# huster-wgm/SRCGAN

Hardware: AMD Instinct MI355X
Metric: paired SR-CycleGAN train images/sec at x4 256->1024 (higher is better)
Workload: dtype bf16; 1 GPU; Sat2Aerx4 paired G+D step (BASELINE configs[1]): 23-block RRDB generator + 3-layer PatchGAN, 3x256x256->3x1024x1024, batch 16/GPU; per_gpu_batch=16, global_batch=16, parallelism=dp1, gradient_exchange=none (1 rank)

## Files before the change

srcgan_amd/csrc/wgrad_dense.hip:

```cpp
#include "common.h"
#include <type_traits>
#include <stdlib.h>

struct WdSeg { int g0, g1; float* grad; float* bias; int Cin; float alpha; };
struct WdP {
    const void* dy; const void* x; float* slab;
    int B, H, W, G, C, dycoff, xcoff;
    long dypix, dyplane, xpix, xplane;
    int g_base;
    int cin_lim[4];
    int nsplit, tiles_x, tiles_y, ntiles, ncit, want_bias;
    unsigned long long* trace;
};
struct WdRedP {
    const float* slab; int nsplit, ncit, COT, g_base, nseg; WdSeg seg[8]; int accumulate;
};

typedef __attribute__((address_space(3))) s16x4 lds_s16x4_;
__device__ __forceinline__ bf16x8 tr_frag2(const char* p0, const char* p1) {
    s16x4 lo = __builtin_amdgcn_ds_read_tr16_b64_v4i16((lds_s16x4_*)(p0));
    s16x4 hi = __builtin_amdgcn_ds_read_tr16_b64_v4i16((lds_s16x4_*)(p1));
    typedef __attribute__((ext_vector_type(8))) short s16x8;
    s16x8 v = {lo[0], lo[1], lo[2], lo[3], hi[0], hi[1], hi[2], hi[3]};
    return __builtin_bit_cast(bf16x8, v);
}

static __device__ __attribute__((aligned(64))) unsigned int wd_zero_page[16];
template <typename T>
__device__ __forceinline__ size_t wd_chan_off(int c, long plane) {
    constexpr int KCE = DT<T>::KCE;
    return (size_t)(c / KCE) * plane + (size_t)(c % KCE) * sizeof(T);
}
typedef const __attribute__((address_space(1))) void* wd_gptr_t;
typedef __attribute__((address_space(3))) void* wd_lptr_t;

template <typename T, int MT, int NT, int TH>
__global__ __launch_bounds__(MT * NT * 64) void wgrad_dense_k(const WdP p) {
    using D = DT<T>;
    constexpr int NW = MT * NT, TW = 32, NTAP = 9;
    constexpr int IHT = TH + 2, IWT = TW + 2;
    constexpr int PB = 32 * (int)sizeof(T), PPP = PB / 16, PXP = 64 / PPP;
    constexpr int DPX = TH * TW, XPX = IHT * IWT;
    constexpr int DPP = (DPX + PXP - 1) / PXP, XPP = (XPX + PXP - 1) / PXP;
    constexpr int DBYTES = DPP * 1024, XBYTES = XPP * 1024;
    constexpr int NPIECE = MT * DPP + NT * XPP, SBYTES = MT * DBYTES + NT * XBYTES;
    constexpr int IPW = (NPIECE + NW - 1) / NW;
    extern __shared__ __attribute__((aligned(1024))) char smem[];

    const int tid = threadIdx.x, lane = tid & 63, wave = tid >> 6, r = lane & 31, h = lane >> 5;
    const int wm = wave / NT, wn = wave % NT;
    const int cit = blockIdx.x, split = blockIdx.y;
    const bool do_bias = wn == 0 && cit == 0 && p.want_bias;
    const char* zp = (const char*)wd_zero_page;

    f32x16 acc[NTAP + 1];
#pragma unroll
    for (int a = 0; a <= NTAP; ++a)
#pragma unroll
        for (int i = 0; i < 16; ++i) acc[a][i] = 0.f;

    const int t_begin = (int)((long)p.ntiles * split / p.nsplit);
    const int t_end = (int)((long)p.ntiles * (split + 1) / p.nsplit);

    auto issue = [&](int t, int stage) {
        int q = t;
        const int tx = q % p.tiles_x; q /= p.tiles_x;
        const int ty = q % p.tiles_y;
        const int b = q / p.tiles_y;
        const int oy0 = ty * TH, ox0 = tx * TW;
        const char* dyb = (const char*)p.dy + (size_t)b * p.H * p.W * p.dypix;
        const char* xb = (const char*)p.x + (size_t)b * p.H * p.W * p.xpix;
        char* ls = smem + stage * SBYTES;
#pragma unroll
        for (int it = 0; it < IPW; ++it) {
            const int pi = it * NW + wave;
            if (IPW * NW != NPIECE && pi >= NPIECE) continue;
            const char* src = zp;
            const int part = lane % PPP, lpx = lane / PPP;
            if (pi < MT * DPP) {
                const int m = pi / DPP, pix = (pi - m * DPP) * PXP + lpx;
                const int oy = oy0 + pix / TW, ox = ox0 + pix % TW;
                const int ch = p.g_base + m * 32 + part * D::EPP;
                if (pix < DPX && oy < p.H && ox < p.W && ch < p.G)
                    src = dyb + (size_t)(oy * p.W + ox) * p.dypix + wd_chan_off<T>(p.dycoff + ch, p.dyplane);
            } else {
                const int pj = pi - MT * DPP, n = pj / XPP, pix = (pj - n * XPP) * PXP + lpx;
                const int iy = pix / IWT, ix = pix - iy * IWT;
                const int gy = oy0 - 1 + iy, gx = ox0 - 1 + ix;
                const int ch = (cit * NT + n) * 32 + part * D::EPP;
                if (pix < XPX && (unsigned)gy < (unsigned)p.H && (unsigned)gx < (unsigned)p.W && ch < p.C)
                    src = xb + (size_t)(gy * p.W + gx) * p.xpix + wd_chan_off<T>(p.xcoff + ch, p.xplane);
            }
            __builtin_amdgcn_global_load_lds((wd_gptr_t)src, (wd_lptr_t)(ls + pi * 1024), 16, 0, 0);
        }
    };

    if (t_begin < t_end) issue(t_begin, 0);
    int stage = 0;
    for (int t = t_begin; t < t_end; ++t, stage ^= 1) {
        __syncthreads();
        if (t + 1 < t_end) issue(t + 1, stage ^ 1);
        const char* my_d = smem + stage * SBYTES + wm * DBYTES;
        const char* my_x = smem + stage * SBYTES + MT * DBYTES + wn * XBYTES;
        if constexpr (std::is_same<T, float>::value) {
#pragma unroll 2
            for (int kk = 0; kk < TH * TW / 2; ++kk) {
                const int pix = 2 * kk + h;
                const int py = pix / TW, px = pix % TW;
                const float a = *(const float*)(my_d + pix * PB + r * 4);
#pragma unroll
                for (int tap = 0; tap < NTAP; ++tap) {
                    const int ky = tap / 3, kx = tap % 3;
                    const float bv = *(const float*)(my_x + ((py + ky) * IWT + px + kx) * PB + r * 4);
                    acc[tap] = __builtin_amdgcn_mfma_f32_32x32x2f32(a, bv, acc[tap], 0, 0, 0);
                }
                if (do_bias) acc[NTAP] = __builtin_amdgcn_mfma_f32_32x32x2f32(a, 1.0f, acc[NTAP], 0, 0, 0);
            }
        } else {
            const int gq = lane >> 4, idx = lane & 15, qq = idx >> 2, pp = idx & 3;
            const int choff = ((gq & 1) * 16 + 4 * pp) * 2;
            const bf16x8 ones = sg_ones16<T>();
#pragma unroll 2
            for (int kk = 0; kk < TH * 2; ++kk) {
                const int py = kk >> 1, xh = (kk & 1) * 16;
                const int px0 = xh + 8 * h + qq;
                const char* ab = my_d + (py * TW + px0) * PB + choff;
                const bf16x8 a = tr_frag2(ab, ab + 4 * PB);
#pragma unroll
                for (int tap = 0; tap < NTAP; ++tap) {
                    const int ky = tap / 3, kx = tap % 3;
                    const char* bb = my_x + ((py + ky) * IWT + px0 + kx) * PB + choff;
                    acc[tap] = sg_mfma16<T>(a, tr_frag2(bb, bb + 4 * PB), acc[tap]);
                }
                if (do_bias) acc[NTAP] = sg_mfma16<T>(a, ones, acc[NTAP]);
            }
        }
    }

    constexpr int COT = 32 * MT, CIT = 32 * NT;
    float* sp = p.slab + ((size_t)split * p.ncit + cit) * (NTAP + 1) * COT * CIT;
#pragma unroll
    for (int tap = 0; tap <= NTAP; ++tap) {
        if (tap == NTAP && !do_bias) continue;
#pragma unroll
        for (int i = 0; i < 16; ++i) {
            const int row = wm * 32 + 8 * (i >> 2) + 4 * h + (i & 3);
            sp[((size_t)tap * COT + row) * CIT + wn * 32 + r] = acc[tap][i];
        }
    }
}

typedef int wd_v4i __attribute__((ext_vector_type(4)));
__device__ __forceinline__ void wd_dma16(const void* base, int voff, int soff, wd_lptr_t lds) {
    const unsigned long long a = (unsigned long long)base;
    wd_v4i rs;
    rs[0] = __builtin_amdgcn_readfirstlane((int)(a & 0xffffffffu));
    rs[1] = __builtin_amdgcn_readfirstlane((int)((a >> 32) & 0xffffu));
    rs[2] = 0x7fffffff;
    rs[3] = 0x00020000;
    const unsigned dst = __builtin_amdgcn_readfirstlane((unsigned)(unsigned long long)lds);
    unsigned keep;
    asm volatile("s_mov_b32 %0, m0\n\ts_mov_b32 m0, %3\n\ts_nop 0\n\tbuffer_load_dwordx4 %1, %2, %4 offen lds\n\ts_mov_b32 m0, %0"
                 : "=&s"(keep) : "v"(voff), "s"(rs), "s"(dst), "s"(soff) : "memory");
}

#ifndef SG_WD_EXP
#define SG_WD_EXP 0
#endif
template <typename T, int MT, int NT, int TH>
__global__ __launch_bounds__(MT * NT * 64) void wgrad_dense_fast_k(const WdP p) {
    using D = DT<T>;
    constexpr int NW = MT * NT, TW = 32, NTAP = 9;
    constexpr int IHT = TH + 2, IWT = TW + 2;
    constexpr int PB = 64, PXP = 16;
    constexpr int DPX = TH * TW, XPX = IHT * IWT;
    constexpr int DPP = (DPX + PXP - 1) / PXP, XPP = (XPX + PXP - 1) / PXP;
    constexpr int DBYTES = DPP * 1024, XBYTES = XPP * 1024;
    constexpr int NPIECE = MT * DPP + NT * XPP, SBYTES = MT * DBYTES + NT * XBYTES;
    constexpr int IPW = (NPIECE + NW - 1) / NW;
    constexpr int OOB = 0x7fffffff;
#ifndef SG_WD_PPK
#define SG_WD_PPK 0
#endif
    constexpr int PPK = SG_WD_PPK ? SG_WD_PPK : 4;
    static_assert(IPW <= 16, "piece classes are packed 4 bits each into two registers");
    extern __shared__ __attribute__((aligned(1024))) char smem[];

    const int tid = threadIdx.x, lane = tid & 63, r = lane & 31, h = lane >> 5;
    const int wave = __builtin_amdgcn_readfirstlane(tid >> 6);
    const int wm = wave / NT, wn = wave % NT;
    int cit, split;
    {
        const int L = blockIdx.x + gridDim.x * blockIdx.y, nwg = gridDim.x * gridDim.y;
        const int xcd = L & 7, j = L >> 3;
        const int full = (nwg >> 3) * 8;
        const int per = nwg >> 3;
        const int pos = L < full ? xcd * per + j : L;
        cit = pos % p.ncit; split = pos / p.ncit;
        if (split >= p.nsplit) return;
    }
    const bool do_bias = wn == 0 && cit == 0 && p.want_bias;
#ifdef SG_WD_NO_SKIP
    const bool useful = true;
#else
    const bool useful = (cit * NT + wn) * 32 < p.cin_lim[wm] || do_bias;
#endif

#ifndef SG_WD_S16
#define SG_WD_S16 1
#endif
    constexpr bool S16 = SG_WD_S16 != 0;
    int voff[IPW]; long soff[IPW];
    unsigned cls[2] = {0u, 0u};
    {
        const int part = lane & 3, lpx = lane >> 2;
#pragma unroll
        for (int it = 0; it < IPW; ++it) {
            const int pi = it * NW + wave;
            int v = OOB; long so = 0;
            if (pi < MT * DPP) {
                const int m = pi / DPP, pix = (pi - m * DPP) * PXP + lpx;
                const int psw = S16 ? part ^ ((((pix % TW) >> 3) & 1) << 1) : part;
                const int ch = p.g_base + m * 32 + psw * D::EPP;
                if (pix < DPX && ch < p.G) v = ((pix / TW) * p.W + pix % TW) * (int)p.dypix + psw * 16;
                so = (long)wd_chan_off<T>(p.dycoff + p.g_base + m * 32, p.dyplane);
            } else if (pi < NPIECE) {
                const int pj = pi - MT * DPP, n = pj / XPP, pix = (pj - n * XPP) * PXP + lpx;
                const int iy = pix / IWT, ix = pix - iy * IWT;
                const int psw = S16 ? part ^ (((ix >> 3) & 1) << 1) : part;
                const int ch = (cit * NT + n) * 32 + psw * D::EPP;
                if (pix < XPX && ch < p.C) v = (iy * p.W + ix) * (int)p.xpix + psw * 16;
                so = (long)wd_chan_off<T>(p.xcoff + (cit * NT + n) * 32, p.xplane);
                cls[it / 8] |= (unsigned)((iy == 0) | ((iy == IHT - 1) << 1) | ((ix == 0) << 2) | ((ix == IWT - 1) << 3)) << (4 * (it % 8));
            }
            voff[it] = v;
            soff[it] = ((long)__builtin_amdgcn_readfirstlane((int)(so >> 32)) << 32) | (unsigned)__builtin_amdgcn_readfirstlane((int)(so & 0xffffffff));
        }
    }

    f32x16 acc[S16 ? 1 : NTAP + 1];
    f32x4 acq[S16 ? NTAP + 1 : 1][2][2];
#pragma unroll
    for (int a = 0; a < (S16 ? 1 : NTAP + 1); ++a)
#pragma unroll
        for (int i = 0; i < 16; ++i) acc[a][i] = 0.f;
#pragma unroll
    for (int a = 0; a < (S16 ? NTAP + 1 : 1); ++a)
#pragma unroll
        for (int i = 0; i < 16; ++i) acq[a][(i >> 3) & 1][(i >> 2) & 1][i & 3] = 0.f;

    const int t_begin = (int)((long)p.ntiles * split / p.nsplit);
    const int t_end = (int)((long)p.ntiles * (split + 1) / p.nsplit);
    int ty = t_begin % p.tiles_y, tx = (t_begin / p.tiles_y) % p.tiles_x, tb = t_begin / (p.tiles_x * p.tiles_y);
    tx = __builtin_amdgcn_readfirstlane(tx); ty = __builtin_amdgcn_readfirstlane(ty); tb = __builtin_amdgcn_readfirstlane(tb);
    const char* dyo = nullptr; const char* xo = nullptr; unsigned clm[2] = {0u, 0u};
    auto origin = [&]() {
        const long px = ((long)tb * p.H + ty * TH) * p.W + tx * TW;
        dyo = (const char*)p.dy + px * p.dypix;
        xo = (const char*)p.x + (px - p.W - 1) * p.xpix;
        const unsigned m = (unsigned)((ty == 0) | ((ty == p.tiles_y - 1) << 1) | ((tx == 0) << 2) | ((tx == p.tiles_x - 1) << 3));
        clm[0] = cls[0] & (m * 0x11111111u); clm[1] = cls[1] & (m * 0x11111111u);
    };
    auto advance = [&]() { if (++ty == p.tiles_y) { ty = 0; if (++tx == p.tiles_x) { tx = 0; ++tb; } } };
    auto piece = [&](int it, int stage) __attribute__((always_inline)) {
        const int pi = it * NW + wave;
        if (IPW * NW != NPIECE && pi >= NPIECE) return;
        int v = ((clm[it / 8] >> (4 * (it % 8))) & 15u) ? OOB : voff[it];
        if (SG_WD_EXP & 8) v = OOB;
        wd_dma16((pi < MT * DPP ? dyo : xo) + soff[it], v, 0, (wd_lptr_t)(smem + stage * SBYTES + pi * 1024));
    };

    if (t_begin < t_end) {
        origin();
#pragma unroll
        for (int it = 0; it < IPW; ++it) piece(it, 0);
    }
    const int gq = lane >> 4, idx = lane & 15, qq = idx >> 2, pp = idx & 3;
    const int choff = ((gq & 1) * 16 + 4 * pp) * 2;
    const bf16x8 ones = sg_ones16<T>();
    int stage = 0;
    for (int t = t_begin; t < t_end; ++t, stage ^= 1) {
#ifdef SG_TRACE
        const unsigned long long t_arr = __builtin_amdgcn_s_memrealtime();
        __builtin_amdgcn_s_waitcnt(0x0f70);
        const unsigned long long t_land = __builtin_amdgcn_s_memrealtime();
#endif
        __builtin_amdgcn_s_waitcnt(0x0f70);
        __syncthreads();
#ifdef SG_TRACE
        if (p.trace && blockIdx.x == 1 && blockIdx.y == 3 && lane == 0 && t - t_begin >= 8 && t - t_begin < 12)
            p.trace[160 + (t - t_begin - 8) * 8 + wave] = t_arr;
        if (p.trace && blockIdx.x == 1 && blockIdx.y == 3 && wave == 0 && lane == 0 && t - t_begin < 40) {
            p.trace[(t - t_begin) * 4 + 0] = t_arr; p.trace[(t - t_begin) * 4 + 1] = t_land; p.trace[(t - t_begin) * 4 + 2] = __builtin_amdgcn_s_memrealtime();
            p.trace[(t - t_begin) * 4 + 3] = __builtin_readcyclecounter();
        }
#endif
        const bool more = t + 1 < t_end;
        if (more) { advance(); origin(); }
        if (!useful) {
            if (more && !(SG_WD_EXP & 1)) {
#pragma unroll
                for (int it = 0; it < IPW; ++it) piece(it, stage ^ 1);
            }
            continue;
        }
        const char* my_d = smem + stage * SBYTES + wm * DBYTES;
        const char* my_x = smem + stage * SBYTES + MT * DBYTES + wn * XBYTES;
#ifndef SG_WD_PD
#define SG_WD_PD 4
#endif
        if constexpr (S16) {
            constexpr int NG = IHT * 3, PDG = 1;
            bf16x8 fa[TH][2], fb[PDG + 1][2];
            const int kq = lane >> 4;
            const int lb = (8 * kq + qq) * PB + (kq & 1) * 32 + 8 * pp;
            const int mk1 = qq + 1 >= 4 ? 32 : 0, mk2 = qq + 2 >= 4 ? 32 : 0;
            auto rd_b = [&](int G) {
                const int i2 = G / 3, kx = G % 3;
                const char* bb = my_x + (i2 * IWT + kx) * PB;
                const int l0 = lb, l1 = lb ^ (kx == 0 ? 0 : kx == 1 ? mk1 : mk2);
                fb[G % (PDG + 1)][0] = tr_frag2(bb + l0, bb + 4 * PB + l1);
                fb[G % (PDG + 1)][1] = tr_frag2(bb + (l0 ^ 32), bb + 4 * PB + (l1 ^ 32));
            };
            auto rd_a = [&](int py) {
                const char* ab = my_d + py * TW * PB;
                fa[py][0] = tr_frag2(ab + lb, ab + 4 * PB + lb);
                fa[py][1] = tr_frag2(ab + (lb ^ 32), ab + 4 * PB + (lb ^ 32));
            };
            rd_a(0); rd_b(0);
#pragma unroll
            for (int G = 0; G < NG; ++G) {
                const int i2 = G / 3, kx = G % 3;
                if (kx == 1 && i2 + 1 < TH) rd_a(i2 + 1);
                if (G + PDG < NG) rd_b(G + PDG);
                if (more) {
#pragma unroll
                    for (int j = 0; j < 2 * PPK; ++j)
                        if (2 * PPK * G + j < IPW) piece(2 * PPK * G + j, stage ^ 1);
                }
                __builtin_amdgcn_sched_barrier(0);
#pragma unroll
                for (int py = 0; py < TH; ++py) {
                    const int ky = i2 - py;
                    if (ky < 0 || ky > 2) continue;
#pragma unroll
                    for (int mb = 0; mb < 2; ++mb)
#pragma unroll
                        for (int nb = 0; nb < 2; ++nb)
                            acq[ky * 3 + kx][mb][nb] = sg_mfma16s<T>(fa[py][mb], fb[G % (PDG + 1)][nb], acq[ky * 3 + kx][mb][nb]);
                }
                if (do_bias && kx == 0 && (i2 == 0 || i2 >= IHT - 2))
#pragma unroll
                    for (int py = (i2 == 0 ? 0 : i2 == IHT - 2 ? 1 : TH / 2); py < (i2 == 0 ? 1 : i2 == IHT - 2 ? TH / 2 : TH); ++py)
#pragma unroll
                        for (int mb = 0; mb < 2; ++mb) acq[NTAP][mb][0] = sg_mfma16s<T>(fa[py][mb], ones, acq[NTAP][mb][0]);
                __builtin_amdgcn_sched_barrier(0);
            }
        } else {
        constexpr int NGRP = IHT * 3 * 2, PD = SG_WD_PD;
        bf16x8 fa[TH][2], fb[PD + 1];
        auto read_b = [&](int G) {
            const int i2 = G / 6, kx = (G % 6) / 2, xh = G % 2;
            const char* bb = my_x + (i2 * IWT + xh * 16 + 8 * h + qq + kx) * PB + choff;
            fb[G % (PD + 1)] = tr_frag2(bb, bb + 4 * PB);
        };
        auto read_a = [&](int py, int xh) {
            const char* ab = my_d + (py * TW + xh * 16 + 8 * h + qq) * PB + choff;
            fa[py][xh] = tr_frag2(ab, ab + 4 * PB);
        };
        read_a(0, 0); read_b(0); read_a(0, 1);
#pragma unroll
        for (int G = 1; G < PD; ++G) read_b(G);
        constexpr int FA_LEAD = 4;
#ifndef SG_WD_PRIO_K
#define SG_WD_PRIO_K 0
#endif
#pragma unroll
        for (int G = 0; G < NGRP; ++G) {
            if (SG_WD_PRIO_K > 0 && wave >= NW / 2) {
                if (G == 0) __builtin_amdgcn_s_setprio(1);
                if (G == SG_WD_PRIO_K) __builtin_amdgcn_s_setprio(0);
            }
            if ((G + FA_LEAD) % 6 < 2 && (G + FA_LEAD) / 6 >= 1 && (G + FA_LEAD) / 6 < TH) read_a((G + FA_LEAD) / 6, (G + FA_LEAD) % 6);
            if (G + PD < NGRP && !(SG_WD_EXP & 4)) read_b(G + PD);
            if (more && !(SG_WD_EXP & 1)) {
#pragma unroll
                for (int j = 0; j < PPK; ++j)
                    if (PPK * G + j < IPW) piece(PPK * G + j, stage ^ 1);
            }
            __builtin_amdgcn_sched_barrier(0);
#ifdef SG_TRACE
            if (G % 5 == 0 && p.trace && blockIdx.x == 1 && blockIdx.y == 3 && lane == 0 && t - t_begin == 10)
                p.trace[192 + wave * 8 + G / 5] = __builtin_amdgcn_s_memrealtime();
#endif
            const int i2 = G / 6, kx = (G % 6) / 2, xh = G % 2;
#pragma unroll
            for (int py = 0; py < TH; ++py) {
                const int ky = i2 - py;
                if (ky < 0 || ky > 2) continue;
                if (!(SG_WD_EXP & 2)) acc[ky * 3 + kx] = sg_mfma16<T>(fa[py][xh], fb[G % (PD + 1)], acc[ky * 3 + kx]);
                else asm volatile("" :: "v"(fa[py][xh]), "v"(fb[G % (PD + 1)]));
            }
            if (do_bias && kx == 0 && (i2 == 0 || i2 >= IHT - 2))
#pragma unroll
                for (int py = (i2 == 0 ? 0 : i2 == IHT - 2 ? 1 : TH / 2); py < (i2 == 0 ? 1 : i2 == IHT - 2 ? TH / 2 : TH); ++py)
                    acc[NTAP] = sg_mfma16<T>(fa[py][xh], ones, acc[NTAP]);
            __builtin_amdgcn_sched_barrier(0);
        }
        }
    }

    constexpr int COT = 32 * MT, CIT = 32 * NT;
    float* sp = p.slab + ((size_t)split * p.ncit + cit) * (NTAP + 1) * COT * CIT;
    const bool blk_needed = (cit * NT + wn) * 32 < p.cin_lim[wm];
#pragma unroll
    for (int tap = 0; tap <= NTAP; ++tap) {
        if (tap == NTAP ? !do_bias : !blk_needed) continue;
        if constexpr (S16) {
#pragma unroll
            for (int mb = 0; mb < 2; ++mb)
#pragma unroll
                for (int nb = 0; nb < 2; ++nb)
#pragma unroll
                    for (int i = 0; i < 4; ++i) {
                        const int row = wm * 32 + mb * 16 + 4 * (lane >> 4) + i;
                        sp[((size_t)tap * COT + row) * CIT + wn * 32 + nb * 16 + (lane & 15)] = acq[tap][mb][tap == NTAP ? 0 : nb][i];
                    }
        } else {
#pragma unroll
            for (int i = 0; i < 16; ++i) {
                const int row = wm * 32 + 8 * (i >> 2) + 4 * h + (i & 3);
                sp[((size_t)tap * COT + row) * CIT + wn * 32 + r] = acc[tap][i];
            }
        }
    }
}

template <int CIT>
__global__ __launch_bounds__(256) void wgrad_dense_reduce_k(const WdRedP p) {
    __shared__ float red[4][64];
    const long per_split = (long)p.ncit * 10 * p.COT * CIT;
    const int el = threadIdx.x & 63, sl = threadIdx.x >> 6;
    const long e = (long)blockIdx.x * 64 + el;
    float s = 0.f;
    bool wanted = false;
    if (e < per_split) {
        long q = e;
        const int col = (int)(q % CIT); q /= CIT;
        const int row = (int)(q % p.COT); q /= p.COT;
        const int tap = (int)(q % 10);
        const int cit = (int)(q / 10);
        const int g = p.g_base + row, ci = cit * CIT + col;
        for (int k = 0; k < p.nseg; ++k) {
            const WdSeg sg = p.seg[k];
            if (g < sg.g0 || g >= sg.g1) continue;
            wanted = tap == 9 ? (sg.bias && cit == 0 && col == 0) : (sg.grad && ci < sg.Cin);
            break;
        }
    }
    if (wanted) {
        float a0 = 0.f, a1 = 0.f, a2 = 0.f, a3 = 0.f;
        int sp = sl;
        for (; sp + 12 < p.nsplit; sp += 16) {
            a0 += p.slab[(size_t)sp * per_split + e];
            a1 += p.slab[(size_t)(sp + 4) * per_split + e];
            a2 += p.slab[(size_t)(sp + 8) * per_split + e];
            a3 += p.slab[(size_t)(sp + 12) * per_split + e];
        }
        for (; sp < p.nsplit; sp += 4) a0 += p.slab[(size_t)sp * per_split + e];
        s = (a0 + a1) + (a2 + a3);
    }
    red[sl][el] = s;
    __syncthreads();
    if (sl != 0 || !wanted) return;
    s = (red[0][el] + red[1][el]) + (red[2][el] + red[3][el]);
    long q = e;
    const int col = (int)(q % CIT); q /= CIT;
    const int row = (int)(q % p.COT); q /= p.COT;
    const int tap = (int)(q % 10);
    const int cit = (int)(q / 10);
    const int g = p.g_base + row, ci = cit * CIT + col;
    for (int k = 0; k < p.nseg; ++k) {
        const WdSeg sg = p.seg[k];
        if (g < sg.g0 || g >= sg.g1) continue;
        const int co = g - sg.g0;
        const float v = s * sg.alpha;
        if (tap == 9) {
            if (sg.bias && cit == 0 && col == 0) sg.bias[co] = p.accumulate ? sg.bias[co] + v : v;
        } else if (sg.grad && ci < sg.Cin) {
            float* gp = sg.grad + ((size_t)co * sg.Cin + ci) * 9 + tap;
            *gp = p.accumulate ? *gp + v : v;
        }
        return;
    }
}

template <typename T, int MT, int NT, int TH>
static int launch_wd(WdP p, hipStream_t st) {
    constexpr int PB = 32 * (int)sizeof(T), PXP = 64 / (PB / 16);
    constexpr size_t SMEM = 2 * 1024 * ((size_t)MT * ((TH * 32 + PXP - 1) / PXP) + (size_t)NT * (((TH + 2) * 34 + PXP - 1) / PXP));
    static_assert(SMEM <= 160 * 1024, "wgrad_dense tile exceeds LDS");
    void (*kern)(const WdP) = wgrad_dense_k<T, MT, NT, TH>;
    bool fast = false;
    if constexpr (!std::is_same<T, float>::value) {
        static const bool no_fast = sg_env("SRCGAN_WD_SLOW") != nullptr;
        const double span_dy = (double)(TH + 2) * p.W * p.dypix, span_x = (double)(TH + 4) * p.W * p.xpix;
        fast = !no_fast && p.H % TH == 0 && p.W % 32 == 0 && span_dy < 2.0e9 && span_x < 2.0e9 &&
               (p.dyplane == 64 || (p.dycoff + p.g_base) % 32 == 0) && (p.xplane == 64 || p.xcoff % 32 == 0);
        constexpr int IPWF = (MT * (TH * 2) + NT * (((TH + 2) * 34 + 15) / 16) + MT * NT - 1) / (MT * NT);
        if constexpr (IPWF <= 10) { if (fast) kern = wgrad_dense_fast_k<T, MT, NT, TH>; }
        else fast = false;
    }
    static bool attr_set[2] = {false, false};
    if (!attr_set[fast]) {
        SG_HIP(hipFuncSetAttribute((const void*)kern, hipFuncAttributeMaxDynamicSharedMemorySize, (int)SMEM));
        attr_set[fast] = true;
    }
    p.tiles_x = cdiv(p.W, 32);
    p.tiles_y = cdiv(p.H, TH);
    p.ntiles = p.B * p.tiles_x * p.tiles_y;
    if (p.nsplit > p.ntiles) p.nsplit = p.ntiles;
    char cls[96];
    snprintf(cls, sizeof(cls), "wgrad_dense<%s,MT%d,NT%d%s>", sizeof(T) == 4 ? "f32" : (__is_same(T, __bf16) ? "bf16" : "f16"), MT, NT, fast ? ",fast" : "");
    const double px = (double)p.B * p.H * p.W;
    const int rows = (p.G - p.g_base) < 32 * MT ? (p.G - p.g_base) : 32 * MT;
    double pairs = 0.0;
    for (int b = 0; b < MT; ++b) {
        const int rb = rows - 32 * b < 32 ? rows - 32 * b : 32;
        if (rb > 0) pairs += (double)rb * (p.cin_lim[b] < p.C ? p.cin_lim[b] : p.C);
    }
    const int tok = sg_prof_start(cls, 2.0 * px * 9 * pairs, px * (rows + p.C) * sizeof(T), st);
#ifdef SG_TRACE
    static unsigned long long* trace = nullptr;
    if (!trace) SG_HIP(hipMalloc(&trace, 64 * 4 * 8));
    SG_HIP(hipMemsetAsync(trace, 0, 64 * 4 * 8, st));
    p.trace = trace;
#endif
    hipLaunchKernelGGL(kern, dim3((unsigned)p.ncit, (unsigned)p.nsplit), dim3(MT * NT * 64), SMEM, st, p);
#ifdef SG_TRACE
    {
        static int dumps = 0;
        if (sg_env("SRCGAN_TRACE") && dumps < 2 && fast) {
            ++dumps;
            unsigned long long h[64 * 4];
            SG_HIP(hipStreamSynchronize(st));
            SG_HIP(hipMemcpy(h, trace, sizeof(h), hipMemcpyDeviceToHost));
            fprintf(stderr, "[trace] %s (10 ns ticks: arrive at barrier, own DMA landed, barrier exit)\n", cls);
            for (int k = 0; k < 4; ++k) {
                fprintf(stderr, "[trace] step %d arrivals by wave (rel. wave 0):", 8 + k);
                for (int w = 0; w < 8; ++w) fprintf(stderr, " %5lld", (long long)(h[160 + k * 8 + w] - h[160 + k * 8]));
                fprintf(stderr, "\n");
            }
            fprintf(stderr, "[trace] step 10: time of groups 0,5,..,35 by wave (rel. wave 0 group 0)\n");
            for (int w = 0; w < 8; ++w) {
                fprintf(stderr, "[trace]   wave %d:", w);
                for (int g = 0; g < 8; ++g) fprintf(stderr, " %5lld", (long long)(h[192 + w * 8 + g] - h[192]));
                fprintf(stderr, "\n");
            }
            for (int k = 0; k < 40 && h[k * 4]; ++k)
                fprintf(stderr, "[trace] %2d arrive %6lld landed %6lld exit %6lld  shader-clock %5.0f MHz\n", k, (long long)(h[k * 4] - h[0]), (long long)(h[k * 4 + 1] - h[0]), (long long)(h[k * 4 + 2] - h[0]),
                        k ? (double)(h[k * 4 + 3] - h[(k - 1) * 4 + 3]) / (double)(h[k * 4 + 2] - h[(k - 1) * 4 + 2]) * 100.0 : 0.0);
        }
    }
#endif
    sg_prof_stop(tok, st);
    SG_LAUNCH_CHECK();
    return p.nsplit;
}

template <typename T>
static int dispatch_wd(const WdP& p, int mt, int nt, hipStream_t st, int& nsplit_used) {
    constexpr bool F = std::is_same<T, float>::value;
    int rc = -1;
    if (nt == 4) {
        if constexpr (!F) {
            switch (mt) {
                case 1: rc = launch_wd<T, 1, 4, 4>(p, st); break;
                case 2: rc = launch_wd<T, 2, 4, 4>(p, st); break;
            }
        }
    } else if (nt == 3) {
        if constexpr (!F) {
            switch (mt) {
                case 1: rc = launch_wd<T, 1, 3, 4>(p, st); break;
                case 2: rc = launch_wd<T, 2, 3, 4>(p, st); break;
            }
        }
    } else
    switch (mt) {
        case 1: rc = launch_wd<T, 1, 2, F ? 2 : 4>(p, st); break;
        case 2: rc = launch_wd<T, 2, 2, F ? 2 : 4>(p, st); break;
        case 3: rc = launch_wd<T, 3, 2, F ? 2 : 4>(p, st); break;
        case 4: rc = launch_wd<T, 4, 2, F ? 2 : 4>(p, st); break;
    }
    if (rc < 0) SG_FAIL("srcgan_wgrad_dense: bad row-tile count %d", mt);
    nsplit_used = rc;
    return 0;
}

static int wd_nt(int mt, int cin_max, int dtype) { return (sg_is16(dtype) && mt <= 2 && cin_max > 64) ? (cin_max <= 96 ? 3 : 4) : 2; }

static int wd_nsplit(int mt, int nt, int ncit, int dtype, int B, int H, int W) {
    const int th = dtype == SRCGAN_F32 ? 2 : 4;
    const int pb = dtype == SRCGAN_F32 ? 128 : 64;
    const long lds = 2 * ((long)mt * th * 32 * pb + (long)nt * (th + 2) * 34 * pb);
    int per_cu = (int)((160 * 1024) / lds); if (per_cu < 1) per_cu = 1;
    if (per_cu * mt * nt > 16) per_cu = 16 / (mt * nt) > 0 ? 16 / (mt * nt) : 1;
    const long ntiles = (long)B * cdiv(H, th) * cdiv(W, 32);
    long cus = 256;
    if (const char* e = sg_env("SRCGAN_WD_CUS")) { const int v = atoi(e); if (v > 0 && v < 256) cus = v; }
    long ns = (cus * per_cu) / ncit;
    if (ns > ntiles) ns = ntiles;
    return (int)(ns < 1 ? 1 : ns);
}

extern "C" size_t srcgan_wgrad_dense_slab_bytes(int G, int C, int dtype, int B, int H, int W) {
    size_t mx = 0;
    for (int g_base = 0; g_base < G; g_base += 128) {
        const int rows = G - g_base < 128 ? G - g_base : 128, mt = cdiv(rows, 32);
        for (int nt = 2; nt <= (sg_is16(dtype) && mt <= 2 ? 4 : 2); ++nt) {
            const int ncit = cdiv(C, 32 * nt);
            const size_t b = (size_t)wd_nsplit(mt, nt, ncit, dtype, B, H, W) * ncit * 10 * (32 * mt) * (32 * nt) * sizeof(float);
            if (b > mx) mx = b;
        }
    }
    return mx;
}

extern "C" int srcgan_wgrad_dense(const srcgan_wgrad_dense_desc* d, void* stream) {
    SG_REQUIRE(d && d->dy && d->x && d->slab, "srcgan_wgrad_dense: null pointer");
    SG_REQUIRE(sg_dtype_ok(d->dtype), "srcgan_wgrad_dense: bad dtype %d", d->dtype);
    const int esz = d->dtype == SRCGAN_F32 ? 4 : 2, epp = 16 / esz;
    SG_REQUIRE(d->B > 0 && d->H > 0 && d->W > 0 && d->G > 0 && d->C > 0 && d->nseg > 0 && d->nseg <= 8,
               "srcgan_wgrad_dense: bad dimensions");
    SG_REQUIRE(d->G % epp == 0 && d->C % epp == 0 && d->dy_cs % epp == 0 && d->dy_coff % epp == 0 && d->x_cs % epp == 0 && d->x_coff % epp == 0,
               "srcgan_wgrad_dense: channel counts/strides/offsets must be multiples of %d", epp);
    SG_REQUIRE((d->dy_plane || d->dy_coff + d->G <= d->dy_cs) && (d->x_plane || d->x_coff + d->C <= d->x_cs), "srcgan_wgrad_dense: channel slice exceeds stride");
    SG_REQUIRE(((uintptr_t)d->x % 16) == 0 && ((uintptr_t)d->dy % 16) == 0, "srcgan_wgrad_dense: tensors must be 16-byte aligned");
    for (int k = 0; k < d->nseg; ++k)
        SG_REQUIRE(d->seg[k].g0 >= 0 && d->seg[k].g1 > d->seg[k].g0 && d->seg[k].g1 <= d->G && d->seg[k].Cin > 0 && d->seg[k].Cin <= d->C,
                   "srcgan_wgrad_dense: bad segment %d", k);
    hipStream_t st = (hipStream_t)stream;
    for (int g_base = 0; g_base < d->G; g_base += 128) {
        const int rows = d->G - g_base < 128 ? d->G - g_base : 128;
        const int mt = cdiv(rows, 32);
        int cin_max = 0, want_bias = 0;
        for (int k = 0; k < d->nseg; ++k)
            if (d->seg[k].g0 < g_base + rows && d->seg[k].g1 > g_base) {
                if (d->seg[k].grad && d->seg[k].Cin > cin_max) cin_max = d->seg[k].Cin;
                if (d->seg[k].bias) want_bias = 1;
            }
        if (cin_max == 0 && !want_bias) continue;
        if (cin_max == 0) cin_max = 1;
        WdP p;
        memset(&p, 0, sizeof(p));
        p.dy = d->dy; p.x = d->x; p.slab = d->slab;
        p.B = d->B; p.H = d->H; p.W = d->W; p.G = d->G; p.C = d->C;
        p.dycoff = d->dy_coff; p.xcoff = d->x_coff;
        p.dypix = (long)d->dy_cs * esz; p.dyplane = d->dy_plane ? d->dy_plane : 64; p.xpix = (long)d->x_cs * esz; p.xplane = d->x_plane ? d->x_plane : 64;
        static const bool nt2_only = sg_env("SRCGAN_WD_NT2") != nullptr;
        const int nt = nt2_only ? 2 : wd_nt(mt, cin_max, d->dtype);
        p.g_base = g_base; p.ncit = cdiv(cin_max, 32 * nt); p.want_bias = want_bias;
        for (int b = 0; b < 4; ++b) {
            p.cin_lim[b] = 0;
            for (int k = 0; k < d->nseg; ++k)
                if (d->seg[k].grad && d->seg[k].g0 < g_base + 32 * (b + 1) && d->seg[k].g1 > g_base + 32 * b && d->seg[k].Cin > p.cin_lim[b])
                    p.cin_lim[b] = d->seg[k].Cin;
        }
        p.nsplit = wd_nsplit(mt, nt, p.ncit, d->dtype, d->B, d->H, d->W);
        int ns = 0;
        if (d->dtype == SRCGAN_F32) SG_TRY(dispatch_wd<float>(p, mt, nt, st, ns));
        else if (d->dtype == SRCGAN_F16) SG_TRY(dispatch_wd<_Float16>(p, mt, nt, st, ns));
        else SG_TRY(dispatch_wd<__bf16>(p, mt, nt, st, ns));
        WdRedP q;
        memset(&q, 0, sizeof(q));
        q.slab = d->slab; q.nsplit = ns; q.ncit = p.ncit; q.COT = 32 * mt; q.g_base = g_base; q.nseg = d->nseg; q.accumulate = d->accumulate;
        for (int k = 0; k < d->nseg; ++k) { q.seg[k].g0 = d->seg[k].g0; q.seg[k].g1 = d->seg[k].g1; q.seg[k].grad = d->seg[k].grad;
                                            q.seg[k].bias = d->seg[k].bias; q.seg[k].Cin = d->seg[k].Cin; q.seg[k].alpha = d->seg[k].alpha; }
        const long per_split = (long)p.ncit * 10 * q.COT * 32 * nt;
        if (nt == 4) hipLaunchKernelGGL(wgrad_dense_reduce_k<128>, dim3((unsigned)cdivl(per_split, 64)), dim3(256), 0, st, q);
        else if (nt == 3) hipLaunchKernelGGL(wgrad_dense_reduce_k<96>, dim3((unsigned)cdivl(per_split, 64)), dim3(256), 0, st, q);
        else hipLaunchKernelGGL(wgrad_dense_reduce_k<64>, dim3((unsigned)cdivl(per_split, 64)), dim3(256), 0, st, q);
        SG_LAUNCH_CHECK();
    }
    return 0;
}
```

Before: 122.0 images/s.

## Add fused triangular wgrad kernel for 192-channel RRDB dense-block weight gradients

Adds a specialised path for the 192x192 dense-block weight-gradient case. It launches one kernel whose workgroups either run the existing fast body on the dense 128-row region or run a new per-wave unit-mapped body covering the irregular triangular remainder. Wave units pick specific (dy block, x block, kx tap) combinations, so only the needed lower-triangular Cin ranges are computed. Previously these ranges were padded per 128-row group across two launches. This adds complex hardcoded unit tables and a shape-specific gate, and it enlarges slab sizing.

```diff
diff --git a/srcgan_amd/csrc/wgrad_dense.hip b/srcgan_amd/csrc/wgrad_dense.hip
--- a/srcgan_amd/csrc/wgrad_dense.hip
+++ b/srcgan_amd/csrc/wgrad_dense.hip
@@ -10,6 +10,7 @@
     int g_base;
     int cin_lim[4];
     int nsplit, tiles_x, tiles_y, ntiles, ncit, want_bias;
+    int slab_ncit;
     unsigned long long* trace;
 };
 struct WdRedP {
@@ -138,7 +139,7 @@
     }
 
     constexpr int COT = 32 * MT, CIT = 32 * NT;
-    float* sp = p.slab + ((size_t)split * p.ncit + cit) * (NTAP + 1) * COT * CIT;
+    float* sp = p.slab + ((size_t)split * p.slab_ncit + cit) * (NTAP + 1) * COT * CIT;
 #pragma unroll
     for (int tap = 0; tap <= NTAP; ++tap) {
         if (tap == NTAP && !do_bias) continue;
@@ -167,8 +168,27 @@
 #ifndef SG_WD_EXP
 #define SG_WD_EXP 0
 #endif
+__device__ __forceinline__ void wd_decode(int L, int nwg, int ncit, int& cit, int& split) {
+    const int xcd = L & 7, j = L >> 3;
+    const int full = (nwg >> 3) * 8;
+    const int per = nwg >> 3;
+    const int pos = L < full ? xcd * per + j : L;
+    cit = pos % ncit; split = pos / ncit;
+}
+
+template <typename T, int MT, int NT, int TH>
+__device__ __forceinline__ void wd_fast_body(const WdP& p, const int cit, const int split);
+
 template <typename T, int MT, int NT, int TH>
 __global__ __launch_bounds__(MT * NT * 64) void wgrad_dense_fast_k(const WdP p) {
+    int cit, split;
+    wd_decode(blockIdx.x + gridDim.x * blockIdx.y, gridDim.x * gridDim.y, p.ncit, cit, split);
+    if (split >= p.nsplit) return;
+    wd_fast_body<T, MT, NT, TH>(p, cit, split);
+}
+
+template <typename T, int MT, int NT, int TH>
+__device__ __forceinline__ void wd_fast_body(const WdP& p, const int cit, const int split) {
     using D = DT<T>;
     constexpr int NW = MT * NT, TW = 32, NTAP = 9;
     constexpr int IHT = TH + 2, IWT = TW + 2;
@@ -189,16 +209,6 @@
     const int tid = threadIdx.x, lane = tid & 63, r = lane & 31, h = lane >> 5;
     const int wave = __builtin_amdgcn_readfirstlane(tid >> 6);
     const int wm = wave / NT, wn = wave % NT;
-    int cit, split;
-    {
-        const int L = blockIdx.x + gridDim.x * blockIdx.y, nwg = gridDim.x * gridDim.y;
-        const int xcd = L & 7, j = L >> 3;
-        const int full = (nwg >> 3) * 8;
-        const int per = nwg >> 3;
-        const int pos = L < full ? xcd * per + j : L;
-        cit = pos % p.ncit; split = pos / p.ncit;
-        if (split >= p.nsplit) return;
-    }
     const bool do_bias = wn == 0 && cit == 0 && p.want_bias;
 #ifdef SG_WD_NO_SKIP
     const bool useful = true;
@@ -411,7 +421,7 @@
     }
 
     constexpr int COT = 32 * MT, CIT = 32 * NT;
-    float* sp = p.slab + ((size_t)split * p.ncit + cit) * (NTAP + 1) * COT * CIT;
+    float* sp = p.slab + ((size_t)split * p.slab_ncit + cit) * (NTAP + 1) * COT * CIT;
     const bool blk_needed = (cit * NT + wn) * 32 < p.cin_lim[wm];
 #pragma unroll
     for (int tap = 0; tap <= NTAP; ++tap) {
@@ -434,6 +444,210 @@
             }
         }
     }
+}
+
+struct WdxType {
+    int g_base, nd, xc0, nx, want_bias;
+    int nsplit;
+    int slab_ncit, slab_cit, COT, CIT;
+    long slab_off;
+    unsigned unit[8];
+};
+struct WdxP {
+    const void* dy; const void* x; float* slab;
+    int B, H, W, G, C, dycoff, xcoff;
+    long dypix, dyplane, xpix, xplane;
+    int tiles_x, tiles_y, ntiles;
+    WdxType ty[2];
+};
+
+template <typename T, int TH>
+__device__ __forceinline__ void wd_kx_body(const WdxP& p, const int type, const int split) {
+    using D = DT<T>;
+    constexpr int NW = 8, TW = 32, NTAP = 9;
+    constexpr int IHT = TH + 2, IWT = TW + 2;
+    constexpr int PB = 64, PXP = 16;
+    constexpr int DPX = TH * TW, XPX = IHT * IWT;
+    constexpr int DPP = (DPX + PXP - 1) / PXP, XPP = (XPX + PXP - 1) / PXP;
+    constexpr int DBYTES = DPP * 1024, XBYTES = XPP * 1024;
+    constexpr int NPMAX = 2 * DPP + 3 * XPP > 3 * DPP + 2 * XPP ? 2 * DPP + 3 * XPP : 3 * DPP + 2 * XPP;
+    constexpr int SBYTES = NPMAX * 1024, IPW = (NPMAX + NW - 1) / NW;
+    constexpr int OOB = 0x7fffffff;
+    static_assert(IPW <= 8, "piece classes are packed 4 bits each into one register");
+    extern __shared__ __attribute__((aligned(1024))) char smem[];
+
+    const int tid = threadIdx.x, lane = tid & 63;
+    const int wave = __builtin_amdgcn_readfirstlane(tid >> 6);
+    const WdxType& tp = p.ty[type];
+    const int nd = tp.nd, npiece = nd * DPP + tp.nx * XPP;
+    const unsigned U = (unsigned)__builtin_amdgcn_readfirstlane((int)tp.unit[wave]);
+    const int m = U & 3, nu = (U >> 2) & 3;
+    const bool do_bias = ((U >> 4) & 1) && tp.want_bias;
+    const int un[2] = {(int)(U >> 8) & 3, (int)(U >> 12) & 3}, ukx[2] = {(int)(U >> 10) & 3, (int)(U >> 14) & 3};
+
+    int voff[IPW]; long soff[IPW];
+    unsigned cls = 0u;
+    {
+        const int part = lane & 3, lpx = lane >> 2;
+#pragma unroll
+        for (int it = 0; it < IPW; ++it) {
+            const int pi = it * NW + wave;
+            int v = OOB; long so = 0;
+            if (pi < nd * DPP) {
+                const int mm = pi / DPP, pix = (pi - mm * DPP) * PXP + lpx;
+                const int psw = part ^ ((((pix % TW) >> 3) & 1) << 1);
+                const int ch = tp.g_base + mm * 32 + psw * D::EPP;
+                if (pix < DPX && ch < p.G) v = ((pix / TW) * p.W + pix % TW) * (int)p.dypix + psw * 16;
+                so = (long)wd_chan_off<T>(p.dycoff + tp.g_base + mm * 32, p.dyplane);
+            } else if (pi < npiece) {
+                const int pj = pi - nd * DPP, n = pj / XPP, pix = (pj - n * XPP) * PXP + lpx;
+                const int iy = pix / IWT, ix = pix - iy * IWT;
+                const int psw = part ^ (((ix >> 3) & 1) << 1);
+                const int ch = tp.xc0 + n * 32 + psw * D::EPP;
+                if (pix < XPX && ch < p.C) v = (iy * p.W + ix) * (int)p.xpix + psw * 16;
+                so = (long)wd_chan_off<T>(p.xcoff + tp.xc0 + n * 32, p.xplane);
+                cls |= (unsigned)((iy == 0) | ((iy == IHT - 1) << 1) | ((ix == 0) << 2) | ((ix == IWT - 1) << 3)) << (4 * it);
+            }
+            voff[it] = v;
+            soff[it] = ((long)__builtin_amdgcn_readfirstlane((int)(so >> 32)) << 32) | (unsigned)__builtin_amdgcn_readfirstlane((int)(so & 0xffffffff));
+        }
+    }
+
+    f32x4 acq[2][3][2][2];
+    f32x4 acb[2];
+#pragma unroll
+    for (int u = 0; u < 2; ++u)
+#pragma unroll
+        for (int i = 0; i < 48; ++i) acq[u][i / 16][(i >> 3) & 1][(i >> 2) & 1][i & 3] = 0.f;
+#pragma unroll
+    for (int i = 0; i < 8; ++i) acb[i >> 2][i & 3] = 0.f;
+
+    const int t_begin = (int)((long)p.ntiles * split / tp.nsplit);
+    const int t_end = (int)((long)p.ntiles * (split + 1) / tp.nsplit);
+    int ty = t_begin % p.tiles_y, tx = (t_begin / p.tiles_y) % p.tiles_x, tb = t_begin / (p.tiles_x * p.tiles_y);
+    tx = __builtin_amdgcn_readfirstlane(tx); ty = __builtin_amdgcn_readfirstlane(ty); tb = __builtin_amdgcn_readfirstlane(tb);
+    const char* dyo = nullptr; const char* xo = nullptr; unsigned clm = 0u;
+    auto origin = [&]() {
+        const long px = ((long)tb * p.H + ty * TH) * p.W + tx * TW;
+        dyo = (const char*)p.dy + px * p.dypix;
+        xo = (const char*)p.x + (px - p.W - 1) * p.xpix;
+        const unsigned mk = (unsigned)((ty == 0) | ((ty == p.tiles_y - 1) << 1) | ((tx == 0) << 2) | ((tx == p.tiles_x - 1) << 3));
+        clm = cls & (mk * 0x11111111u);
+    };
+    auto advance = [&]() { if (++ty == p.tiles_y) { ty = 0; if (++tx == p.tiles_x) { tx = 0; ++tb; } } };
+    auto piece = [&](int it, int stage) __attribute__((always_inline)) {
+        const int pi = it * NW + wave;
+        if (pi >= npiece) return;
+        const int v = ((clm >> (4 * it)) & 15u) ? OOB : voff[it];
+        wd_dma16((pi < nd * DPP ? dyo : xo) + soff[it], v, 0, (wd_lptr_t)(smem + stage * SBYTES + pi * 1024));
+    };
+
+    if (t_begin < t_end) {
+        origin();
+#pragma unroll
+        for (int it = 0; it < IPW; ++it) piece(it, 0);
+    }
+    const int kq = lane >> 4, qq = (lane & 15) >> 2, pp = lane & 3;
+    const int lb = (8 * kq + qq) * PB + (kq & 1) * 32 + 8 * pp;
+    int lx[2];
+#pragma unroll
+    for (int u = 0; u < 2; ++u) lx[u] = lb ^ (ukx[u] == 0 ? 0 : (qq + ukx[u] >= 4 ? 32 : 0));
+    const bf16x8 ones = sg_ones16<T>();
+    int stage = 0;
+    for (int t = t_begin; t < t_end; ++t, stage ^= 1) {
+        __builtin_amdgcn_s_waitcnt(0x0f70);
+        __syncthreads();
+        const bool more = t + 1 < t_end;
+        if (more) { advance(); origin(); }
+        const char* my_d = smem + stage * SBYTES + m * DBYTES;
+        const char* my_x[2];
+#pragma unroll
+        for (int u = 0; u < 2; ++u) my_x[u] = smem + stage * SBYTES + nd * DBYTES + un[u] * XBYTES + ukx[u] * PB;
+        bf16x8 fa[TH][2], fb[2][2];
+        auto rd_a = [&](int py) {
+            const char* ab = my_d + py * TW * PB;
+            fa[py][0] = tr_frag2(ab + lb, ab + 4 * PB + lb);
+            fa[py][1] = tr_frag2(ab + (lb ^ 32), ab + 4 * PB + (lb ^ 32));
+        };
+        auto rd_b = [&](int i2, int u, int slot) {
+            const char* bb = my_x[u] + i2 * IWT * PB;
+            fb[slot][0] = tr_frag2(bb + lb, bb + 4 * PB + lx[u]);
+            fb[slot][1] = tr_frag2(bb + (lb ^ 32), bb + 4 * PB + (lx[u] ^ 32));
+        };
+        auto groups = [&](auto nuc) __attribute__((always_inline)) {
+            constexpr int NU = decltype(nuc)::value;
+            rd_a(0); rd_b(0, 0, 0);
+#pragma unroll
+            for (int G = 0; G < NU * IHT; ++G) {
+                const int i2 = G / NU, u = G % NU;
+                if (u == 0 && i2 + 1 < TH) rd_a(i2 + 1);
+                if (G + 1 < NU * IHT) rd_b((G + 1) / NU, (G + 1) % NU, (G + 1) & 1);
+                if (more && G < 2) {
+#pragma unroll
+                    for (int it = (G == 0 ? 0 : IPW / 2 + 1); it < (G == 0 ? IPW / 2 + 1 : IPW); ++it) piece(it, stage ^ 1);
+                }
+                __builtin_amdgcn_sched_barrier(0);
+#pragma unroll
+                for (int py = 0; py < TH; ++py) {
+                    const int ky = i2 - py;
+                    if (ky < 0 || ky > 2) continue;
+#pragma unroll
+                    for (int mb = 0; mb < 2; ++mb)
+#pragma unroll
+                        for (int nb = 0; nb < 2; ++nb)
+                            acq[u][ky][mb][nb] = sg_mfma16s<T>(fa[py][mb], fb[G & 1][nb], acq[u][ky][mb][nb]);
+                }
+                if (do_bias && u == 0 && i2 < TH)
+#pragma unroll
+                    for (int mb = 0; mb < 2; ++mb) acb[mb] = sg_mfma16s<T>(fa[i2][mb], ones, acb[mb]);
+                __builtin_amdgcn_sched_barrier(0);
+            }
+        };
+        if (nu == 2) groups(std::integral_constant<int, 2>());
+        else groups(std::integral_constant<int, 1>());
+    }
+
+    const int COT = tp.COT, CIT = tp.CIT;
+    float* sp = p.slab + tp.slab_off + ((size_t)split * tp.slab_ncit + tp.slab_cit) * (NTAP + 1) * COT * CIT;
+#pragma unroll
+    for (int u = 0; u < 2; ++u) {
+        if (u >= nu) continue;
+#pragma unroll
+        for (int ky = 0; ky < 3; ++ky)
+#pragma unroll
+            for (int mb = 0; mb < 2; ++mb)
+#pragma unroll
+                for (int nb = 0; nb < 2; ++nb)
+#pragma unroll
+                    for (int i = 0; i < 4; ++i) {
+                        const int row = m * 32 + mb * 16 + 4 * (lane >> 4) + i, col = un[u] * 32 + nb * 16 + (lane & 15);
+                        sp[((size_t)(ky * 3 + ukx[u]) * COT + row) * CIT + col] = acq[u][ky][mb][nb][i];
+                    }
+    }
+    if (do_bias)
+#pragma unroll
+        for (int mb = 0; mb < 2; ++mb)
+#pragma unroll
+            for (int nb = 0; nb < 2; ++nb)
+#pragma unroll
+                for (int i = 0; i < 4; ++i) {
+                    const int row = m * 32 + mb * 16 + 4 * (lane >> 4) + i;
+                    sp[((size_t)NTAP * COT + row) * CIT + nb * 16 + (lane & 15)] = acb[mb][i];
+                }
+}
+
+struct WdTriP { WdP a; WdxP x; int na; };
+template <typename T>
+__global__ __launch_bounds__(512) void wgrad_dense_tri_k(const WdTriP p) {
+    const int L = blockIdx.x;
+    if (L < p.na) {
+        int cit, split;
+        wd_decode(L, p.na, p.a.ncit, cit, split);
+        wd_fast_body<T, 4, 2, 4>(p.a, cit, split);
+        return;
+    }
+    const int j = L - p.na, n0 = p.x.ty[0].nsplit;
+    wd_kx_body<T, 4>(p.x, j < n0 ? 0 : 1, j < n0 ? j : j - n0);
 }
 
 template <int CIT>
@@ -614,6 +828,97 @@
     return (int)(ns < 1 ? 1 : ns);
 }
 
+static constexpr int WD_TRI_C = 192;
+static const int wd_tri_lim[6] = {192, 192, 160, 128, 96, 64};
+static constexpr long WD_TRI_SLAB0 = 3L * 10 * 128 * 64, WD_TRI_SLAB1 = 10L * 64 * 96;
+static void wd_tri_nsplit(int dtype, int B, int H, int W, int& ns0, int& ns1) {
+    ns0 = wd_nsplit(4, 2, 3, dtype, B, H, W);
+    ns1 = wd_nsplit(2, 3, 1, dtype, B, H, W);
+}
+static bool wd_tri_ok(const srcgan_wgrad_dense_desc* d) {
+    static const bool off = sg_env("SRCGAN_WD_SLOW") != nullptr;
+    if (off || !sg_is16(d->dtype) || d->G != WD_TRI_C || d->C != WD_TRI_C || d->H % 4 || d->W % 32) return false;
+    const long dypix = (long)d->dy_cs * 2, xpix = (long)d->x_cs * 2;
+    if ((double)6 * d->W * dypix >= 2.0e9 || (double)8 * d->W * xpix >= 2.0e9) return false;
+    if ((d->dy_plane && d->dy_coff % 32) || (d->x_plane && d->x_coff % 32)) return false;
+    for (int b = 0; b < 6; ++b) {
+        int lim = 0;
+        for (int k = 0; k < d->nseg; ++k)
+            if (d->seg[k].grad && d->seg[k].g0 < 32 * (b + 1) && d->seg[k].g1 > 32 * b && d->seg[k].Cin > lim) lim = d->seg[k].Cin;
+        if (lim != wd_tri_lim[b]) return false;
+    }
+    return true;
+}
+static unsigned wd_unit(int m, int nu, int bias, int n0, int kx0, int n1 = 0, int kx1 = 0) {
+    return (unsigned)(m | nu << 2 | bias << 4 | n0 << 8 | kx0 << 10 | n1 << 12 | kx1 << 14);
+}
+
+template <typename T>
+static int wgrad_dense_tri(const srcgan_wgrad_dense_desc* d, hipStream_t st) {
+    int ns0, ns1;
+    wd_tri_nsplit(d->dtype, d->B, d->H, d->W, ns0, ns1);
+    int want_bias[2] = {0, 0};
+    for (int k = 0; k < d->nseg; ++k)
+        if (d->seg[k].bias) {
+            if (d->seg[k].g0 < 128) want_bias[0] = 1;
+            if (d->seg[k].g1 > 128) want_bias[1] = 1;
+        }
+    WdTriP tp;
+    memset(&tp, 0, sizeof(tp));
+    WdP& a = tp.a;
+    a.dy = d->dy; a.x = d->x; a.slab = d->slab;
+    a.B = d->B; a.H = d->H; a.W = d->W; a.G = d->G; a.C = d->C; a.dycoff = d->dy_coff; a.xcoff = d->x_coff;
+    a.dypix = (long)d->dy_cs * 2; a.dyplane = d->dy_plane ? d->dy_plane : 64; a.xpix = (long)d->x_cs * 2; a.xplane = d->x_plane ? d->x_plane : 64;
+    a.tiles_x = d->W / 32; a.tiles_y = d->H / 4; a.ntiles = d->B * a.tiles_x * a.tiles_y;
+    a.g_base = 0; a.ncit = 2; a.slab_ncit = 3; a.want_bias = want_bias[0]; a.nsplit = ns0;
+    for (int b = 0; b < 4; ++b) a.cin_lim[b] = wd_tri_lim[b];
+    tp.na = 2 * ns0;
+    WdxP& x = tp.x;
+    x.dy = a.dy; x.x = a.x; x.slab = a.slab;
+    x.B = a.B; x.H = a.H; x.W = a.W; x.G = a.G; x.C = a.C; x.dycoff = a.dycoff; x.xcoff = a.xcoff;
+    x.dypix = a.dypix; x.dyplane = a.dyplane; x.xpix = a.xpix; x.xplane = a.xplane;
+    x.tiles_x = a.tiles_x; x.tiles_y = a.tiles_y; x.ntiles = a.ntiles;
+    WdxType& t0 = x.ty[0];
+    t0.g_base = 0; t0.nd = 3; t0.xc0 = 128; t0.nx = 2; t0.want_bias = 0; t0.nsplit = ns0;
+    t0.slab_ncit = 3; t0.slab_cit = 2; t0.COT = 128; t0.CIT = 64; t0.slab_off = 0;
+    const unsigned u0[8] = {wd_unit(0, 2, 0, 0, 0, 0, 1), wd_unit(0, 2, 0, 0, 2, 1, 0), wd_unit(0, 2, 0, 1, 1, 1, 2), wd_unit(2, 2, 0, 0, 0, 0, 1),
+                            wd_unit(1, 2, 0, 0, 0, 0, 1), wd_unit(1, 2, 0, 0, 2, 1, 0), wd_unit(1, 2, 0, 1, 1, 1, 2), wd_unit(2, 1, 0, 0, 2)};
+    WdxType& t1 = x.ty[1];
+    t1.g_base = 128; t1.nd = 2; t1.xc0 = 0; t1.nx = 3; t1.want_bias = want_bias[1]; t1.nsplit = ns1;
+    t1.slab_ncit = 1; t1.slab_cit = 0; t1.COT = 64; t1.CIT = 96; t1.slab_off = (long)ns0 * WD_TRI_SLAB0;
+    const unsigned u1[8] = {wd_unit(0, 2, 0, 0, 0, 0, 1), wd_unit(0, 2, 0, 0, 2, 1, 0), wd_unit(0, 2, 0, 1, 1, 1, 2), wd_unit(0, 1, 1, 2, 2),
+                            wd_unit(0, 2, 0, 2, 0, 2, 1), wd_unit(1, 2, 0, 0, 0, 0, 1), wd_unit(1, 2, 0, 0, 2, 1, 0), wd_unit(1, 2, 1, 1, 1, 1, 2)};
+    for (int w = 0; w < 8; ++w) { t0.unit[w] = u0[w]; t1.unit[w] = u1[w]; }
+    {
+        constexpr int DB = 8 * 1024, XB = 13 * 1024;
+        constexpr size_t SMEM = 2 * (size_t)(4 * DB + 2 * XB);
+        static_assert(SMEM <= 160 * 1024 && 2 * (2 * DB + 3 * XB) <= SMEM, "wgrad_dense_tri tile exceeds LDS");
+        static bool attr_set = false;
+        if (!attr_set) { SG_HIP(hipFuncSetAttribute((const void*)wgrad_dense_tri_k<T>, hipFuncAttributeMaxDynamicSharedMemorySize, (int)SMEM)); attr_set = true; }
+        char cls[64];
+        snprintf(cls, sizeof(cls), "wgrad_dense_tri<%s>", __is_same(T, __bf16) ? "bf16" : "f16");
+        const double px = (double)d->B * d->H * d->W;
+        double pairs = 0.0;
+        for (int b = 0; b < 6; ++b) pairs += 32.0 * wd_tri_lim[b];
+        const int tok = sg_prof_start(cls, 2.0 * px * 9 * pairs, px * (128 + 128 + 5 * 32 + 5 * 32) * sizeof(T), st);
+        hipLaunchKernelGGL((wgrad_dense_tri_k<T>), dim3((unsigned)(2 * ns0 + ns0 + ns1)), dim3(512), SMEM, st, tp);
+        sg_prof_stop(tok, st);
+        SG_LAUNCH_CHECK();
+    }
+    for (int grp = 0; grp < 2; ++grp) {
+        WdRedP q;
+        memset(&q, 0, sizeof(q));
+        q.slab = (const float*)d->slab + (grp ? (size_t)ns0 * WD_TRI_SLAB0 : 0);
+        q.nsplit = grp ? ns1 : ns0; q.ncit = grp ? 1 : 3; q.COT = grp ? 64 : 128; q.g_base = grp ? 128 : 0; q.nseg = d->nseg; q.accumulate = d->accumulate;
+        for (int k = 0; k < d->nseg; ++k) { q.seg[k].g0 = d->seg[k].g0; q.seg[k].g1 = d->seg[k].g1; q.seg[k].grad = d->seg[k].grad;
+                                            q.seg[k].bias = d->seg[k].bias; q.seg[k].Cin = d->seg[k].Cin; q.seg[k].alpha = d->seg[k].alpha; }
+        if (grp) hipLaunchKernelGGL(wgrad_dense_reduce_k<96>, dim3((unsigned)cdivl(WD_TRI_SLAB1, 64)), dim3(256), 0, st, q);
+        else hipLaunchKernelGGL(wgrad_dense_reduce_k<64>, dim3((unsigned)cdivl(WD_TRI_SLAB0, 64)), dim3(256), 0, st, q);
+        SG_LAUNCH_CHECK();
+    }
+    return 0;
+}
+
 extern "C" size_t srcgan_wgrad_dense_slab_bytes(int G, int C, int dtype, int B, int H, int W) {
     size_t mx = 0;
     for (int g_base = 0; g_base < G; g_base += 128) {
@@ -623,6 +928,12 @@
             const size_t b = (size_t)wd_nsplit(mt, nt, ncit, dtype, B, H, W) * ncit * 10 * (32 * mt) * (32 * nt) * sizeof(float);
             if (b > mx) mx = b;
         }
+    }
+    if (sg_is16(dtype) && G == WD_TRI_C && C == WD_TRI_C && H % 4 == 0 && W % 32 == 0) {
+        int ns0, ns1;
+        wd_tri_nsplit(dtype, B, H, W, ns0, ns1);
+        const size_t b = ((size_t)ns0 * WD_TRI_SLAB0 + (size_t)ns1 * WD_TRI_SLAB1) * sizeof(float);
+        if (b > mx) mx = b;
     }
     return mx;
 }
@@ -641,6 +952,7 @@
         SG_REQUIRE(d->seg[k].g0 >= 0 && d->seg[k].g1 > d->seg[k].g0 && d->seg[k].g1 <= d->G && d->seg[k].Cin > 0 && d->seg[k].Cin <= d->C,
                    "srcgan_wgrad_dense: bad segment %d", k);
     hipStream_t st = (hipStream_t)stream;
+    if (wd_tri_ok(d)) return d->dtype == SRCGAN_F16 ? wgrad_dense_tri<_Float16>(d, st) : wgrad_dense_tri<__bf16>(d, st);
     for (int g_base = 0; g_base < d->G; g_base += 128) {
         const int rows = d->G - g_base < 128 ? d->G - g_base : 128;
         const int mt = cdiv(rows, 32);
@@ -660,7 +972,7 @@
         p.dypix = (long)d->dy_cs * esz; p.dyplane = d->dy_plane ? d->dy_plane : 64; p.xpix = (long)d->x_cs * esz; p.xplane = d->x_plane ? d->x_plane : 64;
         static const bool nt2_only = sg_env("SRCGAN_WD_NT2") != nullptr;
         const int nt = nt2_only ? 2 : wd_nt(mt, cin_max, d->dtype);
-        p.g_base = g_base; p.ncit = cdiv(cin_max, 32 * nt); p.want_bias = want_bias;
+        p.g_base = g_base; p.ncit = cdiv(cin_max, 32 * nt); p.slab_ncit = p.ncit; p.want_bias = want_bias;
         for (int b = 0; b < 4; ++b) {
             p.cin_lim[b] = 0;
             for (int k = 0; k < d->nseg; ++k)
```

Result: no change. 123.0 images/s (median of 6 runs) (+0.8%).
